# kofinandi/pixel-nerf-yolo

Hardware: AMD Instinct MI355X
Metric: rays/sec (whole node), 64 samples/ray, 3-view 128×128 render (higher is better)
Workload: dtype f32 (matrix products on f16x2 split operands, fp32 accumulate)

## Files before the change

### pixel-nerf-yolo_amd/csrc/api.hip

```cpp
#include <algorithm>
#include <cmath>
#include <cstdio>
#include <cstdlib>
#include <cstring>
#include <map>
#include <string>
#include <vector>

#include "api_internal.h"

namespace pny {

static thread_local std::string g_err;
void set_error(const std::string& msg) { g_err = msg; }
int hip_fail(hipError_t e, const char* what) {
    g_err = std::string("HIP error: ") + hipGetErrorString(e) + " in " + what;
    return PNY_ERR_HIP;
}
int fail(int code, const std::string& msg) {
    g_err = msg;
    return code;
}

}
// ... 819 lines not shown
        if (v < 0 || v >= d->n_views_all) return fail(PNY_ERR_ARG, who + "view id outside [0, n_views_all)");
        double inv[16];
        if (!invert4(poses_host + 16 * v, inv)) return fail(PNY_ERR_ARG, who + "singular extrinsic matrix");
        for (int r = 0; r < 3; ++r) {
            for (int q = 0; q < 3; ++q) a.pose[i][3 * r + q] = (float)inv[4 * r + q];
            a.pose[i][9 + r] = (float)inv[4 * r + 3];
        }
        a.view_id[i] = (int)v;
    }
    for (int s = 0; s <= d->n_scales; ++s) offsets_host[s] = a.off[s];
    launch_yolo_train_batch(a, (hipStream_t)stream);
    PNY_HIP(hipGetLastError());
    return PNY_OK;
}

}

namespace pny {
static unsigned range_bits(const pny_model* m) {
    return m->range_flag ? __atomic_load_n(m->range_flag, __ATOMIC_RELAXED) : 0u;
}
int check_ready(pny_scene* s, const char* who) {
    if (!s) return fail(PNY_ERR_ARG, std::string(who) + ": null scene");
    if (!s->m->finalized) return fail(PNY_ERR_STATE, std::string(who) + ": weights not finalized (pny_model_finalize)");
    const unsigned bits = s->precision == PNY_PRECISION_F32 ? 0u : range_bits(s->m);
    if (bits) {
        if (bits & PNY_RANGE_WEIGHT) s->m->f16_weights_ok = false;
        return fail(PNY_ERR_RANGE, std::string(who) + ": an earlier f16 (F16X2 / F16) launch left the f16 range (" +
                                       std::string(bits & PNY_RANGE_ACTIVATION ? "activation " : "") +
                                       std::string(bits & PNY_RANGE_GRADIENT ? "gradient " : "") +
                                       std::string(bits & PNY_RANGE_WEIGHT ? "weight " : "") +
                                       "beyond +-65504 or not finite): its results are invalid.  Clear with pny_model_range_status(m, 0, 1), pin "
                                       "pny_scene_set_precision(s, PNY_PRECISION_F32) and repeat the call");
    }
    if (!s->have_latent) return fail(PNY_ERR_STATE, std::string(who) + ": scene has no latent (pny_scene_encode / pny_scene_set_latent)");
    if (!s->have_cams) return fail(PNY_ERR_STATE, std::string(who) + ": scene has no cameras (pny_scene_set_cameras)");
    if (s->cam_ns != s->ns) return fail(PNY_ERR_STATE, std::string(who) + ": camera count != latent view count");
    if (s->n_objs > 1 && s->ns % s->n_objs)
        return fail(PNY_ERR_STATE, std::string(who) + ": grouped scene: the view count is not a multiple of the object count");
    if (obj_views(s) > 1 && s->m->desc.combine_layer >= s->m->desc.n_blocks)
        return fail(PNY_ERR_ARG, std::string(who) + ": multi-view scene needs combine_layer < n_blocks");
    return 0;
}

int view_blocks(const pny_model_desc& d) { return d.combine_layer < d.n_blocks ? d.combine_layer : d.n_blocks; }
}

namespace pny {
double mlp_flops_per_point(const pny_model_desc& d, int ns, MlpPass pass) {
    const int nvb = view_blocks(d);
    const double per_view = (pass == PASS_CHAIN ? 0.0 : (double)d_in(d) * HID) +
                            (pass == PASS_FORWARD ? (double)nvb * d.d_latent * HID : 0.0) + 2.0 * nvb * HID * HID;
    const double post = 2.0 * (d.n_blocks - nvb) * HID * HID + (double)HID * d.d_out;
    return 2.0 * (ns * per_view + post);
}
}

enum MlpKernel { K_F32_8x64 = MLP_8x64, K_F32_16x64 = MLP_16x64, K_F32_8x32 = MLP_8x32, K_H2, K_H2S, K_H1 };
struct MlpRoute {
    MlpKernel kernel;
    Prec prec;
    bool stash;
    bool projected;
    int tile;
    int grid_cap;
};

static bool f16_default(const pny_scene* s) {
    const pny_model* m = s->m;
    return s->precision != PNY_PRECISION_F32 && m->f16_weights_ok && mlp_h2_supports(m->desc.n_blocks, m->desc.combine_layer);
}

static bool wants_projection(const pny_scene* s, long long n_points, bool force) {
    if (!s->m->has_zproj) return false;
    if ((long long)s->hl * s->wl * view_blocks(s->m->desc) * HID >= (1ll << 31)) return false;
    if (force) return true;
    if (s->zp_mode == PNY_PROJECTION_OFF) return false;
    return s->zp_mode != PNY_PROJECTION_AUTO || f16_default(s) || n_points >= 2ll * s->hl * s->wl;
}

static MlpRoute route_mlp(const pny_scene* s, long long n_points, bool stash) {
    const pny_model_desc& d = s->m->desc;
    const int prec = s->precision;
    const bool can_f16 = prec != PNY_PRECISION_F32 && (s->m->f16_weights_ok || prec == PNY_PRECISION_F16X2) &&
                         mlp_h2_supports(d.n_blocks, d.combine_layer) && (!stash || s->L % 128 == 0);
    MlpRoute r;
    r.stash = stash;
    r.projected = stash ? can_f16 && wants_projection(s, n_points, true) : wants_projection(s, n_points, false);
    const bool f16 = r.projected && can_f16;
    const bool h1 = f16 && (prec == PNY_PRECISION_F16_TRAIN || (prec == PNY_PRECISION_F16 && !stash));
    bool h2s = f16 && !h1 && !stash && n_points <= 32ll * mlp_max_grid(MLP_8x64);
    if (f16 && !h1 && !stash)
        if (const char* e = getenv("PNYOLO_H2_SPLIT")) h2s = atoi(e) != 0;
    const int shape = (f16 || stash) ? MLP_8x64 : mlp_pick_variant(n_points);
    r.kernel = h1 ? K_H1 : h2s ? K_H2S : f16 ? K_H2 : MlpKernel(shape);
    r.prec = h1 ? PREC_H1 : f16 ? PREC_H2 : PREC_F32;
    r.tile = h2s ? 32 : mlp_tile_samples(shape);
    r.grid_cap = h2s ? 2 * mlp_max_grid(MLP_8x64) : mlp_max_grid(shape);
    if (!stash)
        if (const char* e = getenv("PNYOLO_GRID")) {
            const int g = atoi(e);
            if (g > 0 && g < r.grid_cap) r.grid_cap = g;
        }
    return r;
}

namespace pny {
// ... 89 lines not shown
    pny_model* m = s->m;
    const pny_model_desc& d = m->desc;
    MlpArgs a;
    int rc;
    if ((rc = fill_mlp_args(s, mode, xyz, dirs, rays, z, K, n_points, coarse, out, &a))) return rc;
    const bool fine_w = !(coarse || !d.has_fine || !m->use_fine);
    const int which = fine_w ? 1 : 0;
    bool room = false;
    if (stash_pass >= 0) {
        s->stashed[stash_pass].valid = false;
        room = m->defer && obj_views(s) == m->defer_ns && m->defer_used[which] + a.n_tiles <= m->defer_cap[which];
    }
    const MlpRoute r = route_mlp(s, n_points, room);
    if (r.stash) {
        pny_scene::StashedPass& sp = s->stashed[stash_pass];
        a.lay = stash_layout(d, obj_views(s), s->L);
        a.stash_x = a.lay.x_record(m->dx_stash[which].f(), m->defer_used[which]);
        sp.valid = true;
        sp.epoch = m->defer_epoch;
        sp.which = which;
        sp.tile0 = m->defer_used[which];
        sp.tiles = a.n_tiles;
        sp.n_points = n_points;
        m->defer_used[which] += a.n_tiles;
    }
    if (r.projected) {
        if ((rc = ensure_projection(s, which, n_points, st, &a.zp, r.stash))) return rc;
        a.tap_stride = a.zp_stride;
    }
    if (r.kernel == K_H1) {
        if ((rc = want_h1_images(m, s->precision == PNY_PRECISION_F16_TRAIN))) return rc;
        use_images(a, f16_images(m, fine_w, true));
    }
    const long long tiles = (n_points + r.tile - 1) / r.tile;
    if (tiles > 0x7fffffffll) return fail(PNY_ERR_ARG, "too many points for one launch");
    a.n_tiles = (int)tiles;
    a.idx32 = (tiles * r.tile) < 0xffffffffll;
    const int grid = (int)std::min<long long>(r.grid_cap, tiles);
    if ((rc = stamp_event(s->timing, s->ev, s->ev_used, st))) return rc;
    switch (r.kernel) {
    case K_H1: (r.stash ? launch_mlp_h1_stash : launch_mlp_h1)(a, grid, st); break;
    case K_H2: (r.stash ? launch_mlp_h2_stash : launch_mlp_h2)(a, grid, st); break;
    case K_H2S: launch_mlp_h2s(a, grid, st); break;
    default:
        if (r.stash)
            launch_mlp_stash(a, grid, st);
        else
            launch_mlp(a, r.kernel, grid, st);
    }
    PNY_HIP(hipGetLastError());
    if ((rc = stamp_event(s->timing, s->ev, s->ev_used, st))) return rc;
    s->last_prec = r.prec;
    s->last_projected = r.projected;
    s->last_flops += mlp_flops_per_point(d, obj_views(s), r.projected ? PASS_FORWARD_PROJECTED : PASS_FORWARD) * (double)n_points;
    s->last_flops_ref += mlp_flops_per_point(d, obj_views(s), PASS_FORWARD) * (double)n_points;
    s->last_launches += 1;
    return 0;
}

static void begin_call(pny_scene* s) {
    s->ev_used = 0;
    s->last_flops = 0.0;
    s->last_flops_ref = 0.0;
    s->last_launches = 0;
}

extern "C" {

int pny_query(pny_scene* s, const float* xyz_dev, const float* viewdirs_dev, int64_t n, int coarse, float* out_dev,
              pny_stream stream) {
    int rc;
    if ((rc = check_ready(s, "pny_query"))) return rc;
    if (n < 0 || (n > 0 && (!xyz_dev || !viewdirs_dev || !out_dev))) return fail(PNY_ERR_ARG, "pny_query: bad argument");
    PNY_HIP(hipSetDevice(s->m->desc.device));
    if ((rc = enter_stream(s, (hipStream_t)stream))) return rc;
    begin_call(s);
    return run_mlp(s, 0, xyz_dev, viewdirs_dev, nullptr, nullptr, 1, n, coarse, out_dev, (hipStream_t)stream);
}

int pny_sample_coarse(const float* rays_dev, int64_t n, int n_coarse, int lindisp, const float* u_dev, uint64_t seed,
                      float* z_dev, pny_stream stream) {
    if (n < 0 || n_coarse < 1 || (n > 0 && (!rays_dev || !z_dev))) return fail(PNY_ERR_ARG, "pny_sample_coarse: bad argument");
    launch_sample_coarse(rays_dev, n, n_coarse, lindisp, u_dev, seed, z_dev, (hipStream_t)stream);
    PNY_HIP(hipGetLastError());
    return PNY_OK;
}

int pny_composite(const float* rays_dev, const float* z_dev, const float* sample_dev, int64_t n, int k, int white_bkgd,
                  float* weights_dev, float* rgb_dev, float* depth_dev, pny_stream stream) {
    if (n < 0 || k < 1 || (n > 0 && (!rays_dev || !z_dev || !sample_dev))) return fail(PNY_ERR_ARG, "pny_composite: bad argument");
    launch_composite(rays_dev, z_dev, sample_dev, n, k, white_bkgd, weights_dev, rgb_dev, depth_dev, (hipStream_t)stream);
    PNY_HIP(hipGetLastError());
    return PNY_OK;
}

int pny_sample_fine(const float* rays_dev, const float* z_coarse_dev, const float* weights_dev, const float* depth_dev,
                    int64_t n, int n_coarse, int n_fine, int n_fine_depth, float depth_std, int lindisp,
                    const float* u_dev, const float* u2_dev, const float* g_dev, uint64_t seed, float* z_out_dev,
                    pny_stream stream) {
    if (n < 0 || n_coarse < 1 || n_fine < 0 || n_fine_depth < 0 || n_fine_depth > n_fine)
        return fail(PNY_ERR_ARG, "pny_sample_fine: bad sample counts");
    if (n > 0 && (!rays_dev || !z_coarse_dev || !weights_dev || !z_out_dev || (n_fine_depth > 0 && !depth_dev)))
        return fail(PNY_ERR_ARG, "pny_sample_fine: null argument");
    if ((size_t)(4 * n_coarse + 1 + 2 * n_fine) * 4 * sizeof(float) > 160 * 1024)
        return fail(PNY_ERR_ARG, "pny_sample_fine: n_coarse + n_fine too large for the LDS-resident sort");
    launch_sample_fine(rays_dev, z_coarse_dev, weights_dev, depth_dev, n, n_coarse, n_fine, n_fine_depth, depth_std,
                       lindisp, u_dev, u2_dev, g_dev, seed, z_out_dev, (hipStream_t)stream);
// ... 197 lines not shown
```

### pixel-nerf-yolo_amd/csrc/api_internal.h

```cpp
#pragma once
#include <map>
#include <string>
#include <vector>

#include "pny_common.h"
#include "encoder.h"

namespace pny {

struct HostTensor {
    std::vector<int64_t> shape;
    std::vector<float> data;
};

struct DevBuf {
    void* p = nullptr;
    size_t bytes = 0;
    int reserve(size_t need) {
        if (need <= bytes) return 0;
        if (p) (void)hipFree(p);
        p = nullptr;
        bytes = 0;
        hipError_t e = hipMalloc(&p, need);
        if (e != hipSuccess) return hip_fail(e, "hipMalloc(workspace)");
// ... 177 lines not shown

struct pny_scene {
    pny_model* m = nullptr;
    int ns = 0, L = 0, hl = 0, wl = 0;
    int width = 0, height = 0;
    bool have_cams = false, have_latent = false;
    int cam_ns = 0;
    int n_objs = 1;
    Cam cams[MAX_VIEWS];
    DevBuf latent, work, scratch, enc_work;
    DevBuf zp[2];
    bool zp_valid[2] = {false, false};
    uint64_t zp_generation = 0;
    int zp_mode = PNY_PROJECTION_AUTO;
    float* latent_grad = nullptr;
    int precision = PNY_PRECISION_AUTO;
    Prec last_prec = PREC_F32;
    Prec last_bwd_prec = PREC_F32;
    bool last_projected = false;
    double last_flops_ref = 0.0;
    bool timing = false;
    std::vector<hipEvent_t> ev;
    int ev_used = 0;
    double last_flops = 0.0;
    int last_launches = 0;
    DevBuf dy_absmax;
    DevBuf lg_fixed, lg_words;
    int last_lg_det = 0;
    DevBuf x_stash, dy_stash, dw_partial, dw_bias, dw_tables, d_samp, out_tmp, dz_tmp, sel_tmp, gdepth_tmp;
    long long sel_count = 0;
    PinnedStage table_stage;
    bool stash_next = false;
    struct StashedPass {
        bool valid = false;
        uint64_t epoch = 0;
        int which = 0;
        long long tile0 = 0, tiles = 0, n_points = 0;
    } stashed[2];
    std::vector<hipEvent_t> bev;
    int bev_used = 0;
    double bwd_flops[3] = {0.0, 0.0, 0.0};
    hipStream_t last_stream = nullptr;
    bool has_last_stream = false;
    hipEvent_t order_ev = nullptr;
    bool order_ev_valid = false;
};


namespace pny {
int enter_stream(pny_scene* s, hipStream_t st);
int check_ready(pny_scene* s, const char* who);
int view_blocks(const pny_model_desc& d);
inline int d_in(const pny_model_desc& d) { return 3 + 6 * d.num_freqs + 3; }
enum MlpPass { PASS_FORWARD, PASS_FORWARD_PROJECTED, PASS_CHAIN };
double mlp_flops_per_point(const pny_model_desc& d, int ns, MlpPass pass);
int want_h1_images(pny_model* m, bool transposed = false);
inline const F16Images& f16_images(const pny_model* m, bool fine, bool single_plane) {
    return single_plane ? m->h1[fine ? 1 : 0] : (fine ? m->fine_t : m->coarse_t).h2;
}
inline int obj_views(const pny_scene* s) { return s->ns / (s->n_objs > 0 ? s->n_objs : 1); }
inline StashLayout stash_layout(const pny_model_desc& d, int ns, int L) { return stash_layout(d.n_blocks, d.combine_layer, ns, L); }
int ensure_projection(pny_scene* s, int which, long long n_points, hipStream_t st, const float** zp, bool force = false);
int fill_mlp_args(pny_scene* s, int mode, const float* xyz, const float* dirs, const float* rays, const float* z, int K,
                  long long n_points, int coarse, float* out, MlpArgs* a);
int latent_levels_check(const char* who, const float* const* maps, const int* channels, const int* h, const int* w, int n_levels, int n,
                        long long* total_channels);
int latent_levels_assemble(const char* who, const float* const* maps, const int* channels, const int* h, const int* w, int n_levels, int n,
                           float* latent_nhwc, hipStream_t st);
}
```

### pixel-nerf-yolo_amd/csrc/mlp.hip

```cpp
#include <cstdlib>
#include <cstring>

#include "mlp_core.h"

namespace pny {

template <class C, bool ZP, bool STASH = false>
__global__ __launch_bounds__(C::THREADS, C::WPS) void pny_mlp_kernel(const MlpArgs a) {
    static_assert(!(STASH && ZP), "the stash variant runs the reference operation order");
    constexpr int NT = C::NT, MT = C::MT, TMc = C::TM;
    extern __shared__ __attribute__((aligned(16))) char smem_raw[];
    float4* act = reinterpret_cast<float4*>(smem_raw);
    float4* tap_tab = reinterpret_cast<float4*>(smem_raw + ACT_KG * TMc * 16);

    const int tid = threadIdx.x, lane = tid & 63, wave = __builtin_amdgcn_readfirstlane(tid >> 6);
    float* slab = a.scratch + (size_t)blockIdx.x * (TMc * HID) + (size_t)wave * (NT * MT * 16 * 64) + 4 * lane;
    const int jz_tot = a.L / 8;
#ifdef PNY_STAMP
    StampCtx st;
    st.tr_n = 0;
    st.wave = wave;
    st.lane = lane;
    for (int i = 0; i < ST_N; ++i) st.acc[i] = 0;
    const unsigned long long st_start = stamp_now();
// ... 167 lines not shown
                sum += x.y * ww.y;
                sum += x.z * ww.z;
                sum += x.w * ww.w;
            }
            sum += a.w.b_out[o];
            if (!a.yolo) {
                if (o < 3)
                    sum = 1.0f / (1.0f + expf(-sum));
                else if (o == 3)
                    sum = fmaxf(sum, 0.f);
            }
            const long long s = tile * TMc + m;
            if (s < a.n_points) a.out[s * a.d_out + o] = sum;
        }
        ST_END(ST_LINOUT);
    }
#ifdef PNY_STAMP
    st.acc[ST_TOTAL] = stamp_now() - st_start;
    if (lane == 0)
        for (int i = 0; i < ST_N; ++i) g_stamp_buf[((size_t)blockIdx.x * C::NW + wave) * ST_N + i] = st.acc[i];
#endif
}

int mlp_cu_count() {
    int dev = 0, cus = 0;
    if (hipGetDevice(&dev) != hipSuccess) return 256;
    if (hipDeviceGetAttribute(&cus, hipDeviceAttributeMultiprocessorCount, dev) != hipSuccess || cus <= 0) return 256;
    return cus;
}

static int forced_variant() {
    static int v = -2;
    if (v == -2) {
        const char* e = getenv("PNYOLO_MLP_VARIANT");
        v = -1;
        if (e && !strcmp(e, "8x64")) v = MLP_8x64;
        if (e && !strcmp(e, "16x64")) v = MLP_16x64;
        if (e && !strcmp(e, "8x32")) v = MLP_8x32;
    }
    return v;
}
int mlp_pick_variant(long long n_points) {
    const int f = forced_variant();
    if (f >= 0) return f;
    const long long cus = mlp_cu_count();
    const long long n64 = (n_points + 63) / 64, n32 = (n_points + 31) / 32;
    const double t64 = (double)((n64 + cus - 1) / cus);
    const long long full = n32 / (2 * cus), rem = n32 % (2 * cus);
    const double t32 = 1.05 * (double)full + (rem == 0 ? 0.0 : (rem <= cus ? 0.55 : 1.05));
    return t32 < t64 ? MLP_8x32 : MLP_8x64;
}
int mlp_tile_samples(int variant) { return variant == MLP_8x32 ? 32 : 64; }
int mlp_max_grid(int variant) { return mlp_cu_count() * (variant == MLP_8x32 ? 2 : 1); }
size_t mlp_scratch_floats() { return (size_t)mlp_cu_count() * 64 * HID; }

template <class C, bool ZP>
static void launch_mlp_t(const MlpArgs& a, int grid, hipStream_t st) {
    static LdsLimit lds;
    (void)lds.raise(C::LDS, pny_mlp_kernel<C, ZP>);
#ifdef PNY_STAMP
    static unsigned long long* dbuf = nullptr;
    const size_t nst = (size_t)grid * C::NW * ST_N;
    if (!dbuf) {
        (void)hipMalloc((void**)&dbuf, (size_t)1024 * 16 * ST_N * sizeof(unsigned long long));
        (void)hipMemcpyToSymbol(HIP_SYMBOL(g_stamp_buf), &dbuf, sizeof(dbuf));
    }
    static unsigned long long* tbuf = nullptr;
    if (!tbuf) {
        (void)hipMalloc((void**)&tbuf, (size_t)TRACE_WAVES * TRACE_N * sizeof(unsigned long long));
        (void)hipMemcpyToSymbol(HIP_SYMBOL(g_trace_buf), &tbuf, sizeof(tbuf));
    }
    (void)hipMemsetAsync(tbuf, 0, (size_t)TRACE_WAVES * TRACE_N * sizeof(unsigned long long), st);
    (void)hipMemsetAsync(dbuf, 0, nst * sizeof(unsigned long long), st);
#endif
    hipLaunchKernelGGL((pny_mlp_kernel<C, ZP>), dim3(grid), dim3(C::THREADS), C::LDS, st, a);
#ifdef PNY_STAMP
    {
        std::vector<unsigned long long> hst(nst);
        (void)hipStreamSynchronize(st);
        (void)hipMemcpy(hst.data(), dbuf, nst * sizeof(unsigned long long), hipMemcpyDeviceToHost);
        double sum[ST_N] = {0};
        for (size_t i = 0; i < nst; ++i) sum[i % ST_N] += (double)hst[i];
        static const char* names[ST_N] = {"total", "gemm", "gather", "prologue", "store+sync", "hsum", "lin_out",
                                          "(sync1", "write", "sync2)"};
        fprintf(stderr, "[pny stamp] waves=%d tile=%d tiles=%d grid=%d:", C::NW, C::TM, a.n_tiles, grid);
        for (int i = 0; i < ST_N; ++i) fprintf(stderr, " %s=%.1f%%", names[i], 100.0 * sum[i] / sum[0]);
        fprintf(stderr, " (mean wave cycles %.3g)\n", sum[0] / ((double)grid * C::NW));
        if (const char* tf = getenv("PNYOLO_TRACE_FILE")) {
            std::vector<unsigned long long> tr((size_t)TRACE_WAVES * TRACE_N);
            (void)hipMemcpy(tr.data(), tbuf, tr.size() * sizeof(unsigned long long), hipMemcpyDeviceToHost);
            if (FILE* f = fopen(tf, "a")) {
                for (int w = 0; w < C::NW; ++w) {
                    for (int e = 0; e < TRACE_N; ++e) fprintf(f, "%llu ", tr[(size_t)w * TRACE_N + e]);
                    fprintf(f, "\n");
                }
                fprintf(f, "#\n");
                fclose(f);
            }
        }
    }
#endif
}

template <class C>
static void launch_mlp_c(const MlpArgs& a, int grid, hipStream_t st) {
    if (a.zp)
        launch_mlp_t<C, true>(a, grid, st);
// ... 21 lines not shown
```

### pixel-nerf-yolo_amd/csrc/mlp_h2.hip

```cpp
#include <cstdlib>
#include <cstring>
#include <cstdio>
#include <vector>

#include "mlp_bwd_core.h"
#include "mlp_h2_core.h"

#if PNY_H2_PLANES == 1
#define PNY_H2_KERNEL pny_mlp_h1_kernel
#elif defined(PNY_H2_SPLIT)
#define PNY_H2_KERNEL pny_mlp_h2s_kernel
#else
#define PNY_H2_KERNEL pny_mlp_h2_kernel
#endif

namespace pny {

#ifdef PNY_H2_STAMP
enum { HS_TOTAL = 0, HS_GEMM, HS_GATHER_WAIT, HS_GATHER, HS_EPI_WAIT, HS_EPI, HS_PROLOGUE, HS_LINOUT, HS_SLAB, HS_REAL, HS_N };
__device__ unsigned long long* g_h2_stamp_buf;
__device__ __forceinline__ unsigned long long h2now() {
    unsigned long long t;
    __builtin_amdgcn_sched_barrier(0);
    asm volatile("s_memtime %0\n\ts_waitcnt lgkmcnt(0)" : "=s"(t)::"memory");
// ... 90 lines not shown
                rmax = fmaxf(fmaxf(rmax, fmaxf(r0, r1)), fmaxf(r2, r3));
                if constexpr (STASH) stash_store(stash, stash_lane, stash_off + (unsigned)(((8 * nt + 2 * q) * TM + 32 * mt) * 16), r0, r1, r2, r3);
#if PNY_H2_PLANES == 1
                (void)s1;
                *reinterpret_cast<h4*>(s0) = cvt4(r0, r1, r2, r3);
#else
                h4 p0, p1;
                split4(r0, r1, r2, r3, p0, p1);
                *reinterpret_cast<h4*>(s0) = p0;
                *reinterpret_cast<h4*>(s1) = p1;
#endif
            }
        }
    }
#ifndef PNY_H2_EXP_NOSYNC
    if (__builtin_expect(!(rmax < 65520.0f), 0)) range_report(range_flag, 1u);
#endif
}

struct SlabRef {
    __amdgpu_buffer_rsrc_t rsrc;
    unsigned lane_off;
};
__device__ __forceinline__ void h2slab_store(const f32x16 (&h)[h2::NT][h2::MT], const SlabRef& sl) {
    using namespace h2;
#pragma unroll
    for (int nt = 0; nt < NT; ++nt)
#pragma unroll
        for (int mt = 0; mt < MT; ++mt)
#pragma unroll
            for (int q = 0; q < 4; ++q) {
                const f32x4 v = {h[nt][mt][4 * q + 0], h[nt][mt][4 * q + 1], h[nt][mt][4 * q + 2], h[nt][mt][4 * q + 3]};
                __builtin_amdgcn_raw_buffer_store_b128(__builtin_bit_cast(u32x4, v), sl.rsrc,
                                                       sl.lane_off + (unsigned)(((nt * MT + mt) * 4 + q) * 64 * 16), 0, 2);
            }
}
__device__ __forceinline__ void h2slab_load(f32x16 (&t)[h2::NT][h2::MT], const SlabRef& sl) {
    using namespace h2;
#pragma unroll
    for (int nt = 0; nt < NT; ++nt)
#pragma unroll
        for (int mt = 0; mt < MT; ++mt)
#pragma unroll
            for (int q = 0; q < 4; ++q) {
                const u32x4 u = __builtin_amdgcn_raw_buffer_load_b128(sl.rsrc, sl.lane_off, (unsigned)(((nt * MT + mt) * 4 + q) * 64 * 16), 2);
                const f32x4 v = __builtin_bit_cast(f32x4, u);
                t[nt][mt][4 * q + 0] = v.x;
                t[nt][mt][4 * q + 1] = v.y;
                t[nt][mt][4 * q + 2] = v.z;
                t[nt][mt][4 * q + 3] = v.w;
            }
}

template <int B>
__device__ __forceinline__ void h2gather_commit(const GatherTaps<h2::C, 2>& g, char* planes, int chunk, int wave, int lane) {
    using namespace h2;
    constexpr int NMB = GatherTaps<C>::NMB, QSTEP = GatherTaps<C>::QSTEP;
    const int m = (wave % NMB) * 8 + (lane & 7);
    char* base = planes + (16 * chunk + (lane >> 4)) * (2 * ROW_BYTES) + m * 16 + 8 * ((lane >> 3) & 1);
#pragma unroll
    for (int i = 0; i < GatherTaps<C>::QPW; ++i) {
        const int qb = wave / NMB + i * QSTEP;
        const float4(&x)[4] = g.x[B][i];
        float2 lo, hi;
        lo.x = __builtin_fmaf(x[3].x, g.w[3], __builtin_fmaf(x[2].x, g.w[2], __builtin_fmaf(x[1].x, g.w[1], x[0].x * g.w[0])));
        lo.y = __builtin_fmaf(x[3].y, g.w[3], __builtin_fmaf(x[2].y, g.w[2], __builtin_fmaf(x[1].y, g.w[1], x[0].y * g.w[0])));
        hi.x = __builtin_fmaf(x[3].z, g.w[3], __builtin_fmaf(x[2].z, g.w[2], __builtin_fmaf(x[1].z, g.w[1], x[0].z * g.w[0])));
        hi.y = __builtin_fmaf(x[3].w, g.w[3], __builtin_fmaf(x[2].w, g.w[2], __builtin_fmaf(x[1].w, g.w[1], x[0].w * g.w[0])));
        char* s0 = base + (4 * qb) * (2 * ROW_BYTES);
        *reinterpret_cast<float2*>(s0) = lo;
        *reinterpret_cast<float2*>(s0 + ROW_BYTES) = hi;
    }
}

template <bool STASH>
__device__ __forceinline__ void h2prologue(const MlpArgs& a, int v, long long tile, char* planes, float4* tap_tab, int tid, unsigned* range_flag,
                                           __amdgpu_buffer_rsrc_t stash = __amdgpu_buffer_rsrc_t(), unsigned stash_xin = 0, float4* tap_raw = nullptr) {
    using namespace h2;
    constexpr int NPART = THREADS / TM;
    const int m = tid % TM, part = tid / TM;
    long long s = tile * TM + m;
    if (s >= a.n_points) s = a.n_points - 1;
    float p[3], d[3];
    load_point(a, s, p, d);
    const Cam cam = a.cams[tile_view_base(a, tile * TM) + v];
    float xr[3], xc[3], vd[3];
#pragma unroll
    for (int i = 0; i < 3; ++i) {
        xr[i] = cam.w2c[4 * i + 0] * p[0] + cam.w2c[4 * i + 1] * p[1] + cam.w2c[4 * i + 2] * p[2];
        xc[i] = xr[i] + cam.w2c[4 * i + 3];
        vd[i] = cam.w2c[4 * i + 0] * d[0] + cam.w2c[4 * i + 1] * d[1] + cam.w2c[4 * i + 2] * d[2];
    }
    float rmax = 0.f;
    for (int g = part; g < D_IN_PAD / 4; g += NPART) {
        const float e0 = input_entry(4 * g + 0, xr, vd, a.freq_factor, a.num_freqs), e1 = input_entry(4 * g + 1, xr, vd, a.freq_factor, a.num_freqs);
        const float e2 = input_entry(4 * g + 2, xr, vd, a.freq_factor, a.num_freqs), e3 = input_entry(4 * g + 3, xr, vd, a.freq_factor, a.num_freqs);
        rmax = fmaxf(fmaxf(rmax, fmaxf(fabsf(e0), fabsf(e1))), fmaxf(fabsf(e2), fabsf(e3)));
#if PNY_H2_PLANES == 1
        if constexpr (STASH) stash_store(stash, (unsigned)((g * TM + m) * 16), stash_xin, e0, e1, e2, e3);
        char* s0 = planes + (g >> 1) * (2 * ROW_BYTES) + m * 16 + 8 * (g & 1);
        *reinterpret_cast<h4*>(s0) = cvt4(e0, e1, e2, e3);
#else
        h4 p0, p1;
        split4(e0, e1, e2, e3, p0, p1);
        if constexpr (STASH) stash_store(stash, (unsigned)((g * TM + m) * 16), stash_xin, e0, e1, e2, e3);
        char* s0 = planes + (g >> 1) * (2 * ROW_BYTES) + m * 16 + 8 * (g & 1);
// ... 19 lines not shown
        uy = uy * cam.fy + cam.cy;
        const float gx = ux * a.sx - 1.0f, gy = uy * a.sy - 1.0f;
        const float ix = ((gx + 1.0f) / 2.0f) * (float)(a.Wl - 1);
        const float iy = ((gy + 1.0f) / 2.0f) * (float)(a.Hl - 1);
        const float x0 = floorf(ix), y0 = floorf(iy);
        const float x1 = x0 + 1.0f, y1 = y0 + 1.0f;
        float wgt[4] = {(x1 - ix) * (y1 - iy), (ix - x0) * (y1 - iy), (x1 - ix) * (iy - y0), (ix - x0) * (iy - y0)};
        const float xs[4] = {x0, x1, x0, x1};
        const float ys[4] = {y0, y0, y1, y1};
        const bool cull = a.yolo && !(xc[2] < 0.0f);
        int offs[4], raw[4];
#pragma unroll
        for (int k = 0; k < 4; ++k) {
            const bool ok = (xs[k] >= 0.f) && (xs[k] <= (float)(a.Wl - 1)) && (ys[k] >= 0.f) && (ys[k] <= (float)(a.Hl - 1));
            offs[k] = raw[k] = 0;
            if (ok) {
                offs[k] = ((int)ys[k] * a.Wl + (int)xs[k]) * a.tap_stride;
                raw[k] = ((int)ys[k] * a.Wl + (int)xs[k]) * a.L;
            } else {
                wgt[k] = wgt[k] * 0.0f;
            }
            if (cull || (a.yolo && (wgt[k] != wgt[k]))) wgt[k] = 0.0f;
        }
        tap_tab[2 * m] = make_float4(__int_as_float(offs[0]), __int_as_float(offs[1]), __int_as_float(offs[2]), __int_as_float(offs[3]));
        tap_tab[2 * m + 1] = make_float4(wgt[0], wgt[1], wgt[2], wgt[3]);
        if constexpr (STASH) {
            tap_raw[2 * m] = make_float4(__int_as_float(raw[0]), __int_as_float(raw[1]), __int_as_float(raw[2]), __int_as_float(raw[3]));
            tap_raw[2 * m + 1] = make_float4(wgt[0], wgt[1], wgt[2], wgt[3]);
        }
    }
}

template <bool STASH>
__global__ __launch_bounds__(h2::THREADS, 2) void PNY_H2_KERNEL(const MlpArgs a) {
    using namespace h2;
    extern __shared__ __attribute__((aligned(16))) char smem_raw[];
    char* planes = smem_raw;
    float4* tap_tab = reinterpret_cast<float4*>(smem_raw + ACT_BYTES);
    float* bias_tab = reinterpret_cast<float*>(smem_raw + ACT_BYTES + TAP_BYTES);
    float4* tap_raw = reinterpret_cast<float4*>(smem_raw + lds_bytes(a.n_blocks));
    const int tid = threadIdx.x, lane = tid & 63, wave = __builtin_amdgcn_readfirstlane(tid >> 6);
#ifdef PNY_H2_EXP_STAGGER
    unsigned* sync_cnt = reinterpret_cast<unsigned*>(smem_raw + lds_bytes(a.n_blocks) + TAP_BYTES);
    unsigned sync_epoch = 0;
    if (tid < 2) sync_cnt[tid] = 0;
    __syncthreads();
    if (wave >= 4) {
        const unsigned long long t0 = __builtin_amdgcn_s_memtime();
        while (__builtin_amdgcn_s_memtime() - t0 < (unsigned long long)(PNY_H2_EXP_STAGGER)) __builtin_amdgcn_s_sleep(8);
    }
#endif
    const SlabRef slab = {__builtin_amdgcn_make_buffer_rsrc(a.scratch + (size_t)blockIdx.x * (TM * HID), 0, TM * HID * 4, 0x00020000),
                          (unsigned)((wave * (NT * MT * 16 * 64) + 4 * lane) * 4)};
    const int nb = a.n_blocks;
    const int nvb = a.combine_layer < nb ? a.combine_layer : nb;
    const WStream ws = wstream(a, lane);
    const H2Seg s_in = h2seg(ws, a.h2_in, D_IN_PAD / 16, wave);
#ifdef PNY_H2_EXP_FOOT
    auto fc0seg = [&](int b) { return h2seg(ws, a.h2_fc0[0], HID / 16, wave); };
    auto fc1seg = [&](int b) { return h2seg(ws, a.h2_fc0[0], HID / 16, wave); };
#else
    auto fc0seg = [&](int b) { return h2seg(ws, a.h2_fc0[b], HID / 16, wave); };
    auto fc1seg = [&](int b) { return h2seg(ws, a.h2_fc1[b], HID / 16, wave); };
#endif
    auto entry_bias = [&](int b) -> const float* {
        if constexpr (LDS_BIAS) return bias_tab + (b == 0 ? 0 : 2 * b) * HID;
        return b == 0 ? a.w.b_in : a.w.b_fc1[b - 1];
    };
    auto fc0_bias = [&](int b) -> const float* {
        if constexpr (LDS_BIAS) return bias_tab + (1 + 2 * b) * HID;
        return a.w.b_fc0[b];
    };
    H2Ring ring;
    h2ring_fill(ring, ws, s_in);
#ifdef PNY_H2_STAMP
    unsigned long long hs_acc[HS_N], hs_t_ = 0;
    for (int i = 0; i < HS_N; ++i) hs_acc[i] = 0;
    const unsigned long long hs_start = h2now();
    const unsigned long long hs_real0 = __builtin_amdgcn_s_memrealtime();
#endif
    if constexpr (LDS_BIAS) {
        for (int i = tid; i < (1 + 2 * nb) * HID; i += THREADS) {
            const int vec = i / HID, f = i % HID;
            const float* src = vec == 0 ? a.w.b_in : ((vec & 1) ? a.w.b_fc0[(vec - 1) >> 1] : a.w.b_fc1[(vec - 2) >> 1]);
            bias_tab[i] = src[f];
        }
    }

    const bool xcd_order = (gridDim.x & 7) == 0;
    const long long t_chunk = xcd_order ? (a.n_tiles + 7) / 8 : a.n_tiles;
    const long long t_first = xcd_order ? (long long)(blockIdx.x & 7) * t_chunk + (blockIdx.x >> 3) : blockIdx.x;
    const long long t_last = xcd_order ? ((long long)((blockIdx.x & 7) + 1) * t_chunk < a.n_tiles
                                              ? (long long)((blockIdx.x & 7) + 1) * t_chunk : (long long)a.n_tiles)
                                       : (long long)a.n_tiles;
    const int t_step = xcd_order ? (int)(gridDim.x >> 3) : (int)gridDim.x;
    for (long long tile = t_first; tile < t_last; tile += t_step) {
        f32x16 h[NT][MT];
        f32x16 net[NT][MT];
        GatherTaps<C, 2> g;
        __amdgpu_buffer_rsrc_t xr = __amdgpu_buffer_rsrc_t();
        if constexpr (STASH)
            xr = stash_rsrc(a.lay.x_record(a.stash_x, tile), a.lay.x_tile);
        auto block_tail = [&](int blk, const H2Seg& after, bool slab_in, int next_c0, unsigned stash_net) {
            HS_T0();
            h2zero<NT, MT>(net);
            H2SYNC();
            HS_LAP(HS_EPI_WAIT);
            h2gemm(net, ring, ws, fc0seg(blk), fc1seg(blk), planes, lane);
            HS_LAP(HS_GEMM);
            H2SYNC();
            HS_LAP(HS_EPI_WAIT);
            h2epilogue<false, STASH>(net, fc0_bias(blk), planes, wave, lane, a.range_flag, xr, stash_net);
            if (slab_in) {
                h2slab_load(net, slab);
                HS_LAP(HS_EPI);
                H2SYNC();
                HS_LAP(HS_EPI_WAIT);
                h2gemm(h, ring, ws, fc1seg(blk), after, planes, lane);
                HS_LAP(HS_GEMM);
#pragma unroll
                for (int nt = 0; nt < NT; ++nt)
#pragma unroll
                    for (int mt = 0; mt < MT; ++mt)
#pragma unroll
                        for (int r = 0; r < 16; ++r) h[nt][mt][r] = net[nt][mt][r] + h[nt][mt][r];
            } else if (next_c0 >= 0) {
                HS_LAP(HS_EPI);
                H2SYNC();
                HS_LAP(HS_EPI_WAIT);
                h2gemm(h, ring, ws, fc1seg(blk), after, planes, lane, [&]() { gather_issue<C, 0>(g, next_c0, wave); });
                HS_LAP(HS_GEMM);
            } else {
                HS_LAP(HS_EPI);
                H2SYNC();
                HS_LAP(HS_EPI_WAIT);
                h2gemm(h, ring, ws, fc1seg(blk), after, planes, lane);
                HS_LAP(HS_GEMM);
            }
        };
        for (int v = 0; v < a.NS; ++v) {
            const int vb = tile_view_base(a, tile * TM);
            const H2Seg after_view = v + 1 < a.NS ? s_in : (nvb < nb ? fc0seg(nvb) : s_in);
            const unsigned x_view = STASH ? stash_bytes((unsigned)v * (unsigned)a.lay.x_view) : 0u;
            auto act_slot = [&](int i) { return x_view + stash_bytes((unsigned)a.lay.o_act + (unsigned)i * (unsigned)STASH_SLOT); };
            HS_T0();
            H2SYNC_P();
            h2prologue<STASH>(a, v, tile, planes, tap_tab, tid, a.range_flag, xr, x_view + stash_bytes((unsigned)a.lay.o_in), tap_raw);
            h2zero<NT, MT>(h);
            H2SYNC_P();
            if constexpr (STASH) {
                const unsigned xz = x_view + stash_bytes((unsigned)a.lay.o_z);
                gather_setup<C>(g, a.latent + (size_t)(vb + v) * a.Hl * a.Wl * a.L, tap_raw, wave, lane);
                const int nch = a.L / GCH;
                const unsigned zlane = (unsigned)(((lane >> 3) * TM + (wave % 8) * 8 + (lane & 7)) * 16);
                auto put = [&](const float4(&x)[4][4], int c) {
#pragma unroll
                    for (int i = 0; i < 4; ++i) {
                        float4 r;
                        r.x = __builtin_fmaf(x[i][3].x, g.w[3], __builtin_fmaf(x[i][2].x, g.w[2], __builtin_fmaf(x[i][1].x, g.w[1], x[i][0].x * g.w[0])));
                        r.y = __builtin_fmaf(x[i][3].y, g.w[3], __builtin_fmaf(x[i][2].y, g.w[2], __builtin_fmaf(x[i][1].y, g.w[1], x[i][0].y * g.w[0])));
                        r.z = __builtin_fmaf(x[i][3].z, g.w[3], __builtin_fmaf(x[i][2].z, g.w[2], __builtin_fmaf(x[i][1].z, g.w[1], x[i][0].z * g.w[0])));
                        r.w = __builtin_fmaf(x[i][3].w, g.w[3], __builtin_fmaf(x[i][2].w, g.w[2], __builtin_fmaf(x[i][1].w, g.w[1], x[i][0].w * g.w[0])));
                        stash_store(xr, zlane, xz + (unsigned)((32 * c + 8 * i) * TM * 16), r.x, r.y, r.z, r.w);
                    }
                };
                gather_issue<C, 0>(g, 0, wave);
                for (int c = 0; c < nch; c += 2) {
                    if (c + 1 < nch) gather_issue<C, 1>(g, (c + 1) * GCH, wave);
                    __builtin_amdgcn_sched_barrier(0);
                    put(g.x[0], c);
                    if (c + 2 < nch) gather_issue<C, 0>(g, (c + 2) * GCH, wave);
                    __builtin_amdgcn_sched_barrier(0);
                    if (c + 1 < nch) put(g.x[1], c + 1);
                }
            }
            gather_setup<C>(g, a.zp + (size_t)(vb + v) * a.Hl * a.Wl * a.zp_stride, tap_tab, wave, lane);
            gather_issue<C, 0>(g, 0, wave);
            HS_LAP(HS_PROLOGUE);
            h2gemm(h, ring, ws, s_in, fc0seg(0), planes, lane);
            HS_LAP(HS_GEMM);
            auto view_block = [&](int blk, const H2Seg& after, bool slab_in, int next_c0) {
                const int cb = blk * HID;
                HS_LAP(HS_GATHER);
#ifdef PNY_H2_ANOM_VMCNT0
                __builtin_amdgcn_sched_barrier(0);
                asm volatile("s_waitcnt vmcnt(0)" ::: "memory");
                __builtin_amdgcn_sched_barrier(0);
#endif
                H2SYNC();
#ifdef PNY_H2_ANOM_SCHEDBAR
                __builtin_amdgcn_sched_barrier(0);
#endif
                HS_LAP(HS_GATHER_WAIT);
                gather_issue<C, 1>(g, cb + GCH, wave);
                __builtin_amdgcn_sched_barrier(0);
                h2gather_commit<0>(g, planes, 0, wave, lane);
                gather_issue<C, 0>(g, cb + 2 * GCH, wave);
                __builtin_amdgcn_sched_barrier(0);
                h2gather_commit<1>(g, planes, 1, wave, lane);
                gather_issue<C, 1>(g, cb + 3 * GCH, wave);
                __builtin_amdgcn_sched_barrier(0);
                h2gather_commit<0>(g, planes, 2, wave, lane);
                h2gather_commit<1>(g, planes, 3, wave, lane);
                HS_LAP(HS_GATHER);
                H2SYNC();
                HS_LAP(HS_GATHER_WAIT);
                h2epilogue<true, STASH>(h, entry_bias(blk), planes, wave, lane, a.range_flag, xr, act_slot(2 * blk));
                HS_LAP(HS_EPI);
                block_tail(blk, after, slab_in, next_c0, act_slot(2 * blk + 1));
            };
#if defined(PNY_H2_NOPREFETCH)
            for (int blk = 0; blk + 1 < nvb; ++blk) {
                view_block(blk, fc0seg(blk + 1), false, -1);
                gather_issue<C, 0>(g, (blk + 1) * HID, wave);
            }
#else
            for (int blk = 0; blk + 1 < nvb; ++blk) view_block(blk, fc0seg(blk + 1), false, (blk + 1) * HID);
#endif
            view_block(nvb - 1, after_view, v > 0, -1);
            if (a.NS > 1) {
                HS_T0();
                if (v + 1 < a.NS) {
                    h2slab_store(h, slab);
                } else {
                    const float rns = 1.0f / (float)a.NS;
#pragma unroll
                    for (int nt = 0; nt < NT; ++nt)
#pragma unroll
                        for (int mt = 0; mt < MT; ++mt)
#pragma unroll
                            for (int r = 0; r < 16; ++r) h[nt][mt][r] = h[nt][mt][r] * rns;
                }
                HS_LAP(HS_SLAB);
            }
        }
        auto post_slot = [&](int i) { return stash_bytes((unsigned)a.lay.x_post + (unsigned)i * (unsigned)STASH_SLOT); };
        for (int blk = nvb; blk < nb; ++blk) {
            HS_T0();
            H2SYNC();
            HS_LAP(HS_EPI_WAIT);
            h2epilogue<false, STASH>(h, entry_bias(blk), planes, wave, lane, a.range_flag, xr, post_slot(2 * (blk - nvb)));
            HS_LAP(HS_EPI);
            block_tail(blk, blk + 1 < nb ? fc0seg(blk + 1) : s_in, false, -1, post_slot(2 * (blk - nvb) + 1));
        }
        HS_T0();
        H2SYNC();
        h2epilogue<false, STASH>(h, entry_bias(nb), planes, wave, lane, a.range_flag, xr, post_slot(2 * (nb - nvb)));
        H2SYNC();
        for (int idx = tid; idx < a.d_out * TM; idx += THREADS) {
            const int o = idx / TM, m = idx % TM;
            const float4* wrow = reinterpret_cast<const float4*>(a.w.w_out + (size_t)o * HID);
            float sum = 0.f;
#pragma unroll 4
            for (int kg = 0; kg < HID / 8; ++kg) {
                const h8 x0 = *reinterpret_cast<const h8*>(planes + kg * (2 * ROW_BYTES) + m * 16);
#if PNY_H2_PLANES == 1
                const float4 wa = wrow[2 * kg], wb = wrow[2 * kg + 1];
                sum += (float)x0[0] * wa.x;
                sum += (float)x0[1] * wa.y;
                sum += (float)x0[2] * wa.z;
                sum += (float)x0[3] * wa.w;
                sum += (float)x0[4] * wb.x;
                sum += (float)x0[5] * wb.y;
                sum += (float)x0[6] * wb.z;
                sum += (float)x0[7] * wb.w;
#else
                const h8 x1 = *reinterpret_cast<const h8*>(planes + kg * (2 * ROW_BYTES) + ROW_BYTES + m * 16);
                const float4 wa = wrow[2 * kg], wb = wrow[2 * kg + 1];
                sum += ((float)x0[0] + (float)x1[0]) * wa.x;
                sum += ((float)x0[1] + (float)x1[1]) * wa.y;
                sum += ((float)x0[2] + (float)x1[2]) * wa.z;
                sum += ((float)x0[3] + (float)x1[3]) * wa.w;
                sum += ((float)x0[4] + (float)x1[4]) * wb.x;
// ... 81 lines not shown
```

Measured before the change: 202,100.

## Average views before the last view-block fc1 GEMM in the H2 MLP kernel

In the non-stash f16x2 MLP kernel, the last per-view block now sums the post-ReLU fc0 activations and the residual across views in two scratch slabs. It then runs the fc1 GEMM once on the view mean instead of once per view, relying on the linearity of fc1. This removes (NS-1) fc1 GEMMs per tile. The cost is a second scratch slab, extra slab load/store traffic per view pipelined through a small buffer ring, and one extra plane write and sync at the end. The FLOP accounting is updated to match.

```diff
diff --git a/pixel-nerf-yolo_amd/csrc/api.hip b/pixel-nerf-yolo_amd/csrc/api.hip
--- a/pixel-nerf-yolo_amd/csrc/api.hip
+++ b/pixel-nerf-yolo_amd/csrc/api.hip
@@ -895,7 +895,8 @@
     const double per_view = (pass == PASS_CHAIN ? 0.0 : (double)d_in(d) * HID) +
                             (pass == PASS_FORWARD ? (double)nvb * d.d_latent * HID : 0.0) + 2.0 * nvb * HID * HID;
     const double post = 2.0 * (d.n_blocks - nvb) * HID * HID + (double)HID * d.d_out;
-    return 2.0 * (ns * per_view + post);
+    const double once = pass == PASS_FORWARD_VIEW_MEAN ? (double)(ns - 1) * HID * HID : 0.0;
+    return 2.0 * (ns * per_view + post - once);
 }
 }
 
@@ -1091,7 +1092,9 @@
     if ((rc = stamp_event(s->timing, s->ev, s->ev_used, st))) return rc;
     s->last_prec = r.prec;
     s->last_projected = r.projected;
-    s->last_flops += mlp_flops_per_point(d, obj_views(s), r.projected ? PASS_FORWARD_PROJECTED : PASS_FORWARD) * (double)n_points;
+    const bool view_mean = !r.stash && (r.kernel == K_H2 || r.kernel == K_H2S);
+    s->last_flops += mlp_flops_per_point(d, obj_views(s), view_mean ? PASS_FORWARD_VIEW_MEAN : r.projected ? PASS_FORWARD_PROJECTED : PASS_FORWARD) *
+                     (double)n_points;
     s->last_flops_ref += mlp_flops_per_point(d, obj_views(s), PASS_FORWARD) * (double)n_points;
     s->last_launches += 1;
     return 0;
diff --git a/pixel-nerf-yolo_amd/csrc/api_internal.h b/pixel-nerf-yolo_amd/csrc/api_internal.h
--- a/pixel-nerf-yolo_amd/csrc/api_internal.h
+++ b/pixel-nerf-yolo_amd/csrc/api_internal.h
@@ -253,7 +253,7 @@
 int check_ready(pny_scene* s, const char* who);
 int view_blocks(const pny_model_desc& d);
 inline int d_in(const pny_model_desc& d) { return 3 + 6 * d.num_freqs + 3; }
-enum MlpPass { PASS_FORWARD, PASS_FORWARD_PROJECTED, PASS_CHAIN };
+enum MlpPass { PASS_FORWARD, PASS_FORWARD_PROJECTED, PASS_CHAIN, PASS_FORWARD_VIEW_MEAN };
 double mlp_flops_per_point(const pny_model_desc& d, int ns, MlpPass pass);
 int want_h1_images(pny_model* m, bool transposed = false);
 inline const F16Images& f16_images(const pny_model* m, bool fine, bool single_plane) {
diff --git a/pixel-nerf-yolo_amd/csrc/mlp.hip b/pixel-nerf-yolo_amd/csrc/mlp.hip
--- a/pixel-nerf-yolo_amd/csrc/mlp.hip
+++ b/pixel-nerf-yolo_amd/csrc/mlp.hip
@@ -243,7 +243,7 @@
 }
 int mlp_tile_samples(int variant) { return variant == MLP_8x32 ? 32 : 64; }
 int mlp_max_grid(int variant) { return mlp_cu_count() * (variant == MLP_8x32 ? 2 : 1); }
-size_t mlp_scratch_floats() { return (size_t)mlp_cu_count() * 64 * HID; }
+size_t mlp_scratch_floats() { return (size_t)mlp_cu_count() * 64 * HID * 2; }
 
 template <class C, bool ZP>
 static void launch_mlp_t(const MlpArgs& a, int grid, hipStream_t st) {
diff --git a/pixel-nerf-yolo_amd/csrc/mlp_h2.hip b/pixel-nerf-yolo_amd/csrc/mlp_h2.hip
--- a/pixel-nerf-yolo_amd/csrc/mlp_h2.hip
+++ b/pixel-nerf-yolo_amd/csrc/mlp_h2.hip
@@ -166,6 +166,93 @@
             }
 }
 
+#ifndef PNY_H2_SLAB_DEPTH
+#define PNY_H2_SLAB_DEPTH 4
+#endif
+struct SlabPipe {
+    static constexpr int SD = PNY_H2_SLAB_DEPTH;
+    static_assert(SD >= 2, "slab pipeline");
+    f32x4 buf[SD][4];
+};
+__device__ __forceinline__ void h2slab_issue(SlabPipe& sp, int p, const SlabRef& sh, const SlabRef& sr) {
+    const SlabRef& s = (p & 1) ? sh : sr;
+#pragma unroll
+    for (int q = 0; q < 4; ++q)
+        sp.buf[p % SlabPipe::SD][q] =
+            __builtin_bit_cast(f32x4, __builtin_amdgcn_raw_buffer_load_b128(s.rsrc, s.lane_off, (unsigned)(((p >> 1) * 4 + q) * 64 * 16), 2));
+}
+__device__ __forceinline__ void h2view_sum(f32x16 (&net)[h2::NT][h2::MT], f32x16 (&h)[h2::NT][h2::MT], const float* bias, const SlabRef& sh,
+                                           const SlabRef& sr, bool add, bool store, int wave, int lane) {
+    using namespace h2;
+    SlabPipe sp;
+    const float* bl = bias + 32 * NT * wave + 4 * (lane >> 5);
+    constexpr int NP = 2 * NT * MT, SD = SlabPipe::SD;
+    if (add) {
+#pragma unroll
+        for (int p = 0; p + 1 < SD; ++p) h2slab_issue(sp, p, sh, sr);
+    }
+#pragma unroll
+    for (int p = 0; p < NP; ++p) {
+        const int nt = (p >> 1) / MT, mt = (p >> 1) % MT;
+        if (add) {
+            if (p + SD - 1 < NP) h2slab_issue(sp, p + SD - 1, sh, sr);
+            __builtin_amdgcn_sched_barrier(0);
+        }
+        f32x16& t = (p & 1) ? h[nt][mt] : net[nt][mt];
+#pragma unroll
+        for (int q = 0; q < 4; ++q) {
+            if (!(p & 1)) {
+                const float4 b = *reinterpret_cast<const float4*>(bl + 32 * nt + 8 * q);
+                t[4 * q + 0] = relu1(t[4 * q + 0] + b.x);
+                t[4 * q + 1] = relu1(t[4 * q + 1] + b.y);
+                t[4 * q + 2] = relu1(t[4 * q + 2] + b.z);
+                t[4 * q + 3] = relu1(t[4 * q + 3] + b.w);
+            }
+            if (add) {
+#pragma unroll
+                for (int i = 0; i < 4; ++i) t[4 * q + i] = t[4 * q + i] + sp.buf[p % SD][q][i];
+            }
+            if (store) {
+                const SlabRef& s = (p & 1) ? sh : sr;
+                const f32x4 v = {t[4 * q + 0], t[4 * q + 1], t[4 * q + 2], t[4 * q + 3]};
+                __builtin_amdgcn_raw_buffer_store_b128(__builtin_bit_cast(u32x4, v), s.rsrc, s.lane_off + (unsigned)(((p >> 1) * 4 + q) * 64 * 16), 0, 2);
+            }
+        }
+        if (add) __builtin_amdgcn_sched_barrier(0);
+    }
+}
+
+__device__ __forceinline__ void h2mean_planes(const f32x16 (&net)[h2::NT][h2::MT], f32x16 (&h)[h2::NT][h2::MT], float rns, char* planes, int wave,
+                                              int lane, unsigned* range_flag) {
+    using namespace h2;
+    float rmax = 0.f;
+    char* base = planes + (4 * NT * wave) * (2 * ROW_BYTES) + (lane & 31) * 16 + 8 * (lane >> 5);
+#pragma unroll
+    for (int nt = 0; nt < NT; ++nt)
+#pragma unroll
+        for (int mt = 0; mt < MT; ++mt)
+#pragma unroll
+            for (int q = 0; q < 4; ++q) {
+                char* s0 = base + (4 * nt + q) * (2 * ROW_BYTES) + 32 * mt * 16;
+                const float r0 = net[nt][mt][4 * q + 0] * rns, r1 = net[nt][mt][4 * q + 1] * rns;
+                const float r2 = net[nt][mt][4 * q + 2] * rns, r3 = net[nt][mt][4 * q + 3] * rns;
+                rmax = fmaxf(fmaxf(rmax, fmaxf(r0, r1)), fmaxf(r2, r3));
+#if PNY_H2_PLANES == 1
+                *reinterpret_cast<h4*>(s0) = cvt4(r0, r1, r2, r3);
+#else
+                h4 p0, p1;
+                split4(r0, r1, r2, r3, p0, p1);
+                *reinterpret_cast<h4*>(s0) = p0;
+                *reinterpret_cast<h4*>(s0 + ROW_BYTES) = p1;
+#endif
+#pragma unroll
+                for (int i = 0; i < 4; ++i) h[nt][mt][4 * q + i] = h[nt][mt][4 * q + i] * rns;
+            }
+#ifndef PNY_H2_EXP_NOSYNC
+    if (__builtin_expect(!(rmax < 65520.0f), 0)) range_report(range_flag, 1u);
+#endif
+}
+
 template <int B>
 __device__ __forceinline__ void h2gather_commit(const GatherTaps<h2::C, 2>& g, char* planes, int chunk, int wave, int lane) {
     using namespace h2;
@@ -291,6 +378,13 @@
 #endif
     const SlabRef slab = {__builtin_amdgcn_make_buffer_rsrc(a.scratch + (size_t)blockIdx.x * (TM * HID), 0, TM * HID * 4, 0x00020000),
                           (unsigned)((wave * (NT * MT * 16 * 64) + 4 * lane) * 4)};
+#if defined(PNY_H2_PER_VIEW_FC1) || PNY_H2_PLANES == 1
+    constexpr bool VIEW_MEAN = false;
+#else
+    constexpr bool VIEW_MEAN = !STASH;
+#endif
+    const SlabRef slab_r = {__builtin_amdgcn_make_buffer_rsrc(a.scratch + ((size_t)gridDim.x + blockIdx.x) * (TM * HID), 0, TM * HID * 4, 0x00020000),
+                            slab.lane_off};
     const int nb = a.n_blocks;
     const int nvb = a.combine_layer < nb ? a.combine_layer : nb;
     const WStream ws = wstream(a, lane);
@@ -350,7 +444,7 @@
             H2SYNC();
             HS_LAP(HS_EPI_WAIT);
             h2epilogue<false, STASH>(net, fc0_bias(blk), planes, wave, lane, a.range_flag, xr, stash_net);
-            if (slab_in) {
+            if (!VIEW_MEAN && slab_in) {
                 h2slab_load(net, slab);
                 HS_LAP(HS_EPI);
                 H2SYNC();
@@ -418,7 +512,7 @@
             HS_LAP(HS_PROLOGUE);
             h2gemm(h, ring, ws, s_in, fc0seg(0), planes, lane);
             HS_LAP(HS_GEMM);
-            auto view_block = [&](int blk, const H2Seg& after, bool slab_in, int next_c0) {
+            auto block_entry = [&](int blk) {
                 const int cb = blk * HID;
                 HS_LAP(HS_GATHER);
 #ifdef PNY_H2_ANOM_VMCNT0
@@ -446,7 +540,33 @@
                 HS_LAP(HS_GATHER_WAIT);
                 h2epilogue<true, STASH>(h, entry_bias(blk), planes, wave, lane, a.range_flag, xr, act_slot(2 * blk));
                 HS_LAP(HS_EPI);
+            };
+            auto view_block = [&](int blk, const H2Seg& after, bool slab_in, int next_c0) {
+                block_entry(blk);
                 block_tail(blk, after, slab_in, next_c0, act_slot(2 * blk + 1));
+            };
+            auto mean_tail = [&](int blk) {
+                const bool last = v + 1 == a.NS;
+                HS_T0();
+                h2zero<NT, MT>(net);
+                H2SYNC();
+                HS_LAP(HS_EPI_WAIT);
+                h2gemm(net, ring, ws, fc0seg(blk), last ? fc1seg(blk) : s_in, planes, lane);
+                HS_LAP(HS_GEMM);
+                h2view_sum(net, h, fc0_bias(blk), slab, slab_r, v > 0, !last, wave, lane);
+                if (!last) {
+                    HS_LAP(HS_SLAB);
+                    return;
+                }
+                HS_LAP(v > 0 ? HS_SLAB : HS_EPI);
+                H2SYNC();
+                HS_LAP(HS_EPI_WAIT);
+                h2mean_planes(net, h, 1.0f / (float)a.NS, planes, wave, lane, a.range_flag);
+                HS_LAP(HS_EPI);
+                H2SYNC();
+                HS_LAP(HS_EPI_WAIT);
+                h2gemm(h, ring, ws, fc1seg(blk), after_view, planes, lane);
+                HS_LAP(HS_GEMM);
             };
 #if defined(PNY_H2_NOPREFETCH)
             for (int blk = 0; blk + 1 < nvb; ++blk) {
@@ -456,8 +576,13 @@
 #else
             for (int blk = 0; blk + 1 < nvb; ++blk) view_block(blk, fc0seg(blk + 1), false, (blk + 1) * HID);
 #endif
-            view_block(nvb - 1, after_view, v > 0, -1);
-            if (a.NS > 1) {
+            if constexpr (VIEW_MEAN) {
+                block_entry(nvb - 1);
+                mean_tail(nvb - 1);
+            } else {
+                view_block(nvb - 1, after_view, v > 0, -1);
+            }
+            if (!VIEW_MEAN && a.NS > 1) {
                 HS_T0();
                 if (v + 1 < a.NS) {
                     h2slab_store(h, slab);
```

Result: faster. 217,700, median of 6 (+7.7%).
